# bcollico/Deep-Multiview-Depth-Estimation

Measured on AMD Instinct MI355X. Metric: depth maps/sec + warp-kernel HBM GB/s, 3-view 640x512 D=192, 1/2/4/8 GPU, higher is better.
Workload: dtype f32

## Files before the change

deep-multiview-depth-estimation_amd/csrc/capi.hip:

```cpp
#include <algorithm>
#include <cmath>
#include <cstring>

#include "../../include/train/mvs_region_train.h"
#include "launchers.h"

namespace {

using mvs::Geometry;

int check_geometry(int B, int V, int C, int h, int w, int d_count, Geometry& g, int store_es = 0) {
  if (B <= 0 || C <= 0 || h < 2 || w < 2 || d_count <= 0) return MVS_ERR_INVALID_ARGUMENT;
  if (V < 1 || V > MVS_MAX_VIEWS) return MVS_ERR_UNSUPPORTED_VIEWS;
  const uint64_t hw = (uint64_t)h * (uint64_t)w;
  if ((uint64_t)C * hw >= (1ull << 31) || h > 32000 || w > 32000) return MVS_ERR_TOO_LARGE;
  const bool packed = V >= 2 && V <= 8;
  const uint64_t padded = (uint64_t)V * (uint64_t)((C + 3) / 4) * (uint64_t)(h + 2) * (uint64_t)(w + 2) * 16u;
  if (packed && (padded >= (1ull << 31) || 8ull * hw * (uint64_t)store_es >= (1ull << 32))) return MVS_ERR_TOO_LARGE;
  const uint64_t tiles = (hw + mvs::kBlock - 1) / mvs::kBlock;
  const uint64_t total = (uint64_t)B * tiles * (uint64_t)d_count;
  if (total >= (1ull << 31) - 8) return MVS_ERR_TOO_LARGE;
  g.B = B;
  g.V = V;
  g.C = C;
// ... 681 lines not shown
    return MVS_ERR_INVALID_ARGUMENT;
  if (rd <= 0 || rh <= 0 || rw <= 0 || d <= 0 || h <= 0 || w <= 0) return MVS_ERR_INVALID_ARGUMENT;
  if (x0d < 0 || x0h < 0 || x0w < 0 || pd < 0 || ph < 0 || pw < 0) return MVS_ERR_INVALID_ARGUMENT;
  if (!bn_all_or_none(bn_scale, bn_shift, bn_mean)) return MVS_ERR_INVALID_ARGUMENT;
  if ((uint64_t)batch * c_in * rd * rh * rw * 4u >= (1ull << 31)) return MVS_ERR_TOO_LARGE;
  const int layout = (flags & MVS_LAYOUT_CHANNELS_LAST) ? ((flags & MVS_DECONV_WEIGHT_TAPS) ? 3 : 1)
                                                        : ((flags & MVS_DECONV_WEIGHT_TAPS) ? 2 : 0);
  const mvs::LaunchCheck lc;
  mvs::launch_deconv3d_k3s2(x, x2, layout, batch, c_in, rd, rh, rw, x0d, x0h,
                            x0w, weight, d, h, w, pd, ph, pw, bn_scale, bn_shift, bn_mean, residual, y,
                            (hipStream_t)stream);
  return lc.status();
}

int mvs_conv3d_region_fwd(int mode, int flags, const float* x, const float* x2, const float* weight, float* y,
                          int batch, int c_in, int c_out, const int* dims, const int* out_origin,
                          const int* out_size, const int* in_origin, const int* in_size,
                          const int* pad, const float* bn_scale, const float* bn_shift,
                          const float* bn_mean, const unsigned* x_absmax, unsigned* y_bound, void* stream) {
  if (!x || !weight || !y || !dims || !out_origin || !out_size || batch <= 0) return MVS_ERR_INVALID_ARGUMENT;
  if ((uintptr_t)y_bound & 3u) return MVS_ERR_INVALID_ARGUMENT;
  if (mode < MVS_CONV_S1 || mode > MVS_CONV_T2 ||
      (flags & ~(MVS_CONV_OUT_NCDHW | MVS_CONV_IN_C4 | MVS_CONV_IN_BF16 | MVS_CONV_IN_SPLIT | MVS_CONV_PER_LANE |
                 MVS_CONV_S2_LDS)))
    return MVS_ERR_INVALID_ARGUMENT;
  if ((flags & MVS_CONV_S2_LDS) && (flags & MVS_CONV_PER_LANE)) return MVS_ERR_INVALID_ARGUMENT;
  if ((flags & MVS_CONV_IN_BF16) && !(flags & MVS_CONV_IN_C4)) return MVS_ERR_INVALID_ARGUMENT;
  if ((flags & MVS_CONV_IN_SPLIT) && (!(flags & MVS_CONV_IN_C4) || (flags & MVS_CONV_IN_BF16) || !x_absmax ||
                                      ((uintptr_t)x_absmax & 3u)))
    return MVS_ERR_INVALID_ARGUMENT;
  if ((flags & MVS_CONV_IN_C4) && (mode != MVS_CONV_S2 || c_in % 4)) return MVS_ERR_INVALID_ARGUMENT;
  if (mode != MVS_CONV_S2 && (!in_origin || !in_size)) return MVS_ERR_INVALID_ARGUMENT;
  if (!both_or_neither(in_origin, in_size)) return MVS_ERR_INVALID_ARGUMENT;
  const bool boxed = in_origin != nullptr;
  if (mode != MVS_CONV_S1 && !pad) return MVS_ERR_INVALID_ARGUMENT;
  if (((uintptr_t)x | (uintptr_t)x2 | (uintptr_t)weight) & 15u) return MVS_ERR_INVALID_ARGUMENT;
  if (!bn_all_or_none(bn_scale, bn_shift, bn_mean)) return MVS_ERR_INVALID_ARGUMENT;
  uint64_t ovox = (uint64_t)batch, ivox = (uint64_t)batch, nvox = (uint64_t)batch * c_in;
  for (int k = 0; k < 3; ++k) {
    if (dims[k] <= 0 || out_size[k] <= 0 || out_origin[k] < 0 || out_origin[k] + out_size[k] > dims[k])
      return MVS_ERR_INVALID_ARGUMENT;
    if (boxed && (in_size[k] <= 0 || in_origin[k] < 0 || in_origin[k] + in_size[k] > dims[k]))
      return MVS_ERR_INVALID_ARGUMENT;
    ovox *= (uint64_t)out_size[k];
    ivox *= (uint64_t)(boxed ? in_size[k] : dims[k]);
    nvox *= (uint64_t)dims[k];
  }
  uint64_t svox = 1;
  for (int k = 0; k < 3; ++k) svox *= (uint64_t)(boxed ? in_size[k] : dims[k]);
  const uint64_t desc_bytes = mode == MVS_CONV_S2 ? svox * 64u : svox * (uint64_t)c_in * 4u;
  if (ovox >= (1ull << 31) || desc_bytes >= 0xFFFFFFC0ull || ivox * (uint64_t)c_in >= (1ull << 62) ||
      nvox >= (1ull << 62))
    return MVS_ERR_TOO_LARGE;
  const mvs::LaunchCheck lc;
  const int quads = (flags & MVS_CONV_IN_C4)
                        ? ((flags & MVS_CONV_IN_SPLIT) ? 3 : ((flags & MVS_CONV_IN_BF16) ? 2 : 1)) : 0;
  const int st = mvs::launch_conv3d_region(mode, (flags & MVS_CONV_OUT_NCDHW) != 0, quads,
                                           x, x2, weight, y, batch, c_in, c_out, dims, out_origin, out_size,
                                           in_origin, in_size, pad, bn_scale, bn_shift, bn_mean,
                                           (hipStream_t)stream, reinterpret_cast<const uint32_t*>(x_absmax),
                                           reinterpret_cast<uint32_t*>(y_bound), (flags & MVS_CONV_PER_LANE) != 0,
                                           nullptr, nullptr, (flags & MVS_CONV_S2_LDS) != 0);
  if (st != MVS_OK) return st;
  return lc.status();
}

int mvs_conv3d_region_split_weights(const float* weight, int c_in, int c_out, unsigned short* frag, int* weight_exp) {
  if (!weight || !frag || !weight_exp) return MVS_ERR_INVALID_ARGUMENT;
  if (c_out <= 0 || c_out % 16 || !(c_in == 16 || (c_in > 0 && c_in % 32 == 0))) return MVS_ERR_INVALID_ARGUMENT;
  int ew;
  if (!split_scale(weight, (size_t)27 * c_out * c_in, &ew)) return MVS_ERR_INVALID_ARGUMENT;
  const int kbs = mvs::conv3d_region_split_kblocks(c_in), nbs = c_out / 16;
  for (int kb = 0; kb < kbs; ++kb)
    for (int nb = 0; nb < nbs; ++nb)
      for (int lane = 0; lane < 64; ++lane)
        for (int j = 0; j < 8; ++j) {
          const int c = lane & 15, gq = lane >> 4, co = nb * 16 + c;
          int tap, ci;
          if (c_in == 16) {
            tap = 2 * kb + (gq >> 1);
            ci = 8 * (gq & 1) + j;
          } else {
            tap = kb / (c_in / 32);
            ci = (kb % (c_in / 32)) * 32 + 8 * gq + j;
          }
// ... 173 lines not shown
```

deep-multiview-depth-estimation_amd/csrc/conv3d_region.hip:

```cpp
#include <cstdlib>

#include "launchers.h"
#include "region_conv.h"

namespace mvs {
namespace {

struct Geo {
  int n[3];
  int o0[3];
  int on[3];
  int i0[3];
  int in[3];
  int pad[3];
  int out_cf;
  int in_c4;
  const uint32_t* absmax;
  uint32_t* y_bound;
  int st0[3];
  int stn[3];
};

__device__ inline void store_out(float* __restrict__ y, const Geo& g, int b, int co, int vz, int vy, int vx,
                                 int CO, float v) {
  const size_t vox = ((size_t)(vz + g.st0[0]) * g.stn[1] + (vy + g.st0[1])) * g.stn[2] + (vx + g.st0[2]);
  const size_t rvol = (size_t)g.stn[0] * g.stn[1] * g.stn[2];
  if (g.out_cf) y[((size_t)b * CO + co) * rvol + vox] = v;
  else y[((size_t)b * rvol + vox) * CO + co] = v;
}

template <int MODE, int CI, int CO, int RB, int QM, int CLS, int PS = 1>
__device__ __forceinline__ void region_conv(
    const float* __restrict__ x, const float* __restrict__ x2, const float* __restrict__ w,
    float* __restrict__ y, const float* __restrict__ bn_scale, const float* __restrict__ bn_shift,
    const float* __restrict__ bn_mean, const Geo& g) {
  constexpr int NB = CO / 16;
  static_assert(CI % 16 == 0 && CO % 16 == 0, "channel counts in multiples of 16");
  static_assert((MODE == kT2) == (CLS >= 0), "parity classes: transposed convolutions");
  static_assert(PS == 1 || (PS == 4 && CI == 112), "partial sums: the 112-channel input gradient only");
  const int lane = (int)threadIdx.x & 63;
  const int m = lane & 15, kq = lane >> 4;
  const int b = (int)blockIdx.z;

  int cf[3], cn[3];
  constexpr int par[3] = {CLS >= 0 ? (CLS >> 2) & 1 : 0, CLS >= 0 ? (CLS >> 1) & 1 : 0, CLS >= 0 ? CLS & 1 : 0};
  if constexpr (MODE == kT2) {
#pragma unroll
    for (int d = 0; d < 3; ++d) class_dim(g.o0[d], g.on[d], g.pad[d], par[d], cf[d], cn[d]);
  } else {
#pragma unroll
    for (int d = 0; d < 3; ++d) {
      cf[d] = g.o0[d];
      cn[d] = g.on[d];
    }
// ... 27 lines not shown
      else bs[d] = ((o[d] + g.pad[d] - par[d]) >> 1) - g.i0[d];
      unsigned mk = 0;
#pragma unroll
      for (int tt = 0; tt < 3; ++tt) {
        const int dl = MODE == kT2 ? -(tt >> 1) : tt;
        const bool in = ok && bs[d] + dl >= 0 && bs[d] + dl < lim[d] && !(MODE == kT2 && ((tt & 1) != par[d]));
        mk |= in ? (1u << tt) : 0u;
      }
      vm[rb][d] = mk;
    }
    lin[rb] = (bs[0] * lim[1] + bs[1]) * lim[2] + bs[2];
  }

  f4v acc[PS][RB][NB];
#pragma unroll
  for (int ps = 0; ps < PS; ++ps)
#pragma unroll
    for (int rb = 0; rb < RB; ++rb)
#pragma unroll
      for (int nb = 0; nb < NB; ++nb) acc[ps][rb][nb] = f4v{0.0f, 0.0f, 0.0f, 0.0f};

  const size_t rvol = (size_t)g.in[0] * g.in[1] * g.in[2];
  const int sy = lim[2], sz = lim[1] * lim[2];
#pragma unroll
  for (int tz = 0; tz < 3; ++tz) {
    if (MODE == kT2 && ((tz & 1) != par[0])) continue;
#pragma unroll
    for (int ty = 0; ty < 3; ++ty) {
      if (MODE == kT2 && ((ty & 1) != par[1])) continue;
      const int dz = MODE == kT2 ? -(tz >> 1) : tz, dy = MODE == kT2 ? -(ty >> 1) : ty;
      uint32_t vox[3][RB];
#pragma unroll
      for (int tx = 0; tx < 3; ++tx)
#pragma unroll
        for (int rb = 0; rb < RB; ++rb) {
          const int dx = MODE == kT2 ? -(tx >> 1) : tx;
          const bool ok = ((vm[rb][0] >> tz) & (vm[rb][1] >> ty) & (vm[rb][2] >> tx) & 1u) != 0;
          vox[tx][rb] = ok ? (uint32_t)(lin[rb] + dz * sz + dy * sy + dx) : kOob;
        }
#pragma unroll
      for (int cb = 0; cb < CI / 16; ++cb) {
        const int c4 = cb * 16 + kq * 4;
        const int ps = PS == 1 ? 0 : (cb + 1) / 2;
        Rsrc rs, rs2;
        if constexpr (MODE == kS2) {
          if constexpr (QM == 2)
            rs = make_rsrc(reinterpret_cast<const char*>(x) + ((size_t)b * (CI / 4) + cb * 4) * rvol * 8,
                           (uint32_t)(rvol * 32));
          else if constexpr (QM == 1 || QM == 3)
            rs = make_rsrc(x + ((size_t)b * (CI / 4) + cb * 4) * rvol * 4, (uint32_t)(rvol * 64));
          else
            rs = make_rsrc(x + ((size_t)b * CI + cb * 16) * rvol, (uint32_t)(rvol * 64));
        } else {
          rs = make_rsrc(x + (size_t)b * rvol * CI, (uint32_t)(rvol * CI * 4));
          if (x2) rs2 = make_rsrc(x2 + (size_t)b * rvol * CI, (uint32_t)(rvol * CI * 4));
        }
        f4v a[3][RB], bw[3][NB];
#pragma unroll
        for (int tx = 0; tx < 3; ++tx) {
          if (MODE == kT2 && ((tx & 1) != par[2])) continue;
#pragma unroll
          for (int rb = 0; rb < RB; ++rb) {
            const uint32_t vx = vox[tx][rb];
            f4v v;
            if constexpr (MODE == kS2) {
              if constexpr (QM == 2) {
                typedef __attribute__((ext_vector_type(2))) unsigned v2u;
                const v2u p = __builtin_amdgcn_raw_buffer_load_b64(
                    rs, (int)(vx == kOob ? kOob : ((uint32_t)kq * (uint32_t)rvol + vx) * 8u), 0, 0);
                v = f4v{__uint_as_float(p.x << 16), __uint_as_float(p.x & 0xFFFF0000u),
                          __uint_as_float(p.y << 16), __uint_as_float(p.y & 0xFFFF0000u)};
              } else if constexpr (QM == 3) {
                v = unsplit4(__builtin_bit_cast(uint4, __builtin_amdgcn_raw_buffer_load_b128(
                                 rs, (int)(vx == kOob ? kOob : ((uint32_t)kq * (uint32_t)rvol + vx) * 16u), 0, 0)),
                             sx);
              } else if constexpr (QM == 1) {
                v = ld4(rs, vx == kOob ? kOob : ((uint32_t)kq * (uint32_t)rvol + vx) * 16u, 0);
              } else {
#pragma unroll
                for (int q = 0; q < 4; ++q)
                  v[q] = __uint_as_float(__builtin_amdgcn_raw_buffer_load_b32(
                      rs, (int)(vx == kOob ? kOob : ((uint32_t)(kq * 4 + q) * (uint32_t)rvol + vx) * 4u), 0, 0));
              }
            } else {
              const uint32_t eo = vx == kOob ? kOob : (vx * (uint32_t)CI + (uint32_t)c4) * 4u;
              v = ld4(rs, eo, 0);
              if (x2) v += ld4(rs2, eo, 0);
            }
            a[tx][rb] = v;
          }
          const float* wt = w + (size_t)((tz * 3 + ty) * 3 + tx) * CO * CI;
#pragma unroll
          for (int nb = 0; nb < NB; ++nb)
            bw[tx][nb] = *reinterpret_cast<const f4v*>(wt + (size_t)(nb * 16 + m) * CI + c4);
        }
#pragma unroll
        for (int tx = 0; tx < 3; ++tx) {
          if (MODE == kT2 && ((tx & 1) != par[2])) continue;
#pragma unroll
          for (int s = 0; s < 4; ++s)
#pragma unroll
            for (int rb = 0; rb < RB; ++rb)
#pragma unroll
              for (int nb = 0; nb < NB; ++nb)
                acc[ps][rb][nb] =
                    __builtin_amdgcn_mfma_f32_16x16x4f32(a[tx][rb][s], bw[tx][nb][s], acc[ps][rb][nb], 0, 0, 0);
        }
      }
    }
  }

  float vmax = 0.0f;
#pragma unroll
  for (int nb = 0; nb < NB; ++nb) {
    const int co = nb * 16 + m;
    const float sc = bn_scale ? bn_scale[co] : 1.0f, sh = bn_scale ? bn_shift[co] : 0.0f,
                mu = bn_scale ? bn_mean[co] : 0.0f;
#pragma unroll
    for (int rb = 0; rb < RB; ++rb)
#pragma unroll
      for (int r = 0; r < 4; ++r) {
        const int row = row0 + rb * 16 + kq * 4 + r;
        if (row >= rows) continue;
        const int jx = row % cn[2], t = row / cn[2];
        const int jy = t % cn[1], jz = t / cn[1];
        const int vz = cf[0] + step * jz - g.o0[0], vy = cf[1] + step * jy - g.o0[1],
                  vx = cf[2] + step * jx - g.o0[2];
        float v = acc[0][rb][nb][r];
        if constexpr (PS == 4)
          v = (v + acc[1][rb][nb][r]) + (acc[PS - 2][rb][nb][r] + acc[PS - 1][rb][nb][r]);
        if (bn_scale) v = fmaxf((v - mu) * sc + sh, 0.0f);
        vmax = fmaxf(vmax, fabsf(v));
        store_out(y, g, b, co, vz, vy, vx, CO, v);
      }
  }
  if (g.y_bound) bound_update(g.y_bound, vmax);
}

template <int MODE, int CI, int CO, int RB, int QM = 0, int PS = 1>
__global__ __launch_bounds__(kBlock) void conv3d_region_kernel(
    const float* __restrict__ x, const float* __restrict__ x2, const float* __restrict__ w,
    float* __restrict__ y, const float* __restrict__ bn_scale, const float* __restrict__ bn_shift,
    const float* __restrict__ bn_mean, Geo g) {
  if constexpr (MODE == kT2) {
    switch (blockIdx.y) {
#define MVS_T2_CLASS(c) \
  case c: region_conv<MODE, CI, CO, RB, QM, c, PS>(x, x2, w, y, bn_scale, bn_shift, bn_mean, g); break;
      MVS_T2_CLASS(0) MVS_T2_CLASS(1) MVS_T2_CLASS(2) MVS_T2_CLASS(3)
      MVS_T2_CLASS(4) MVS_T2_CLASS(5) MVS_T2_CLASS(6) MVS_T2_CLASS(7)
#undef MVS_T2_CLASS
      default: break;
    }
  } else {
    region_conv<MODE, CI, CO, RB, QM, -1, PS>(x, x2, w, y, bn_scale, bn_shift, bn_mean, g);
  }
}

template <int MODE, int CI, int CO, int RB, int QM = 0, int PS = 1>
void launch_mode(const float* x, const float* x2, const float* w, float* y, const float* sc, const float* sh,
                 const float* mu, int B, const Geo& g, hipStream_t s) {
  hipLaunchKernelGGL((conv3d_region_kernel<MODE, CI, CO, RB, QM, PS>), region_grid(MODE, RB, B, g.on), dim3(kBlock), 0, s,
                     x, x2, w, y, sc, sh, mu, g);
}

template <int CI>
struct S1TileF {
  static constexpr int TZ = CI == 16 ? 8 : (CI == 32 ? 4 : 2);
  static constexpr int PX = 18, PY = 6, PZ = TZ + 2, PV = PX * PY * PZ;
  static constexpr int NCH = CI / 4;
  static constexpr int REC = CI * 4;
  static constexpr int LDS = PV * REC;
};

template <int CI>
__device__ inline int s1f_off(int v, int c) {
  constexpr int NCH = CI / 4;
  return v * (CI * 4) + ((c ^ (((v * NCH) >> 3) % NCH)) << 4);
}

template <int CI, int CO>
__global__ __launch_bounds__(kBlock) void conv3d_s1_lds_kernel(
    const float* __restrict__ x, const float* __restrict__ w, float* __restrict__ y,
    const float* __restrict__ bn_scale, const float* __restrict__ bn_shift, const float* __restrict__ bn_mean, Geo g,
    int tiles_x, int tiles_y, int tiles_z) {
  using T = S1TileF<CI>;
// ... 105 lines not shown
      float v = acc[r][i];
      if (bn_scale) v = fmaxf((v - mu) * sc + sh, 0.0f);
      vmax = fmaxf(vmax, fabsf(v));
      store_out(y, g, b, co, tz0 + zz, ty0 + yy, tx0 + 4 * kq + i, CO, v);
    }
  }
  if (g.y_bound) bound_update(g.y_bound, vmax);
}

template <int CI>
void launch_s1_lds(const float* x, const float* w, float* y, const float* sc, const float* sh, const float* mu,
                   int B, const Geo& g, hipStream_t s) {
  const int tx = (g.on[2] + 15) / 16, ty = (g.on[1] + 3) / 4, tz = (g.on[0] + S1TileF<CI>::TZ - 1) / S1TileF<CI>::TZ;
  hipLaunchKernelGGL((conv3d_s1_lds_kernel<CI, CI>), tile_grid(tx * ty * tz, B), dim3(kBlock), 0, s, x, w, y, sc, sh,
                     mu, g, tx, ty, tz);
}

}

int launch_conv3d_region(int mode, bool out_cf, int in_c4, const float* x, const float* x2, const float* w,
                         float* y, int B, int CI, int CO, const int* n, const int* o0, const int* on, const int* i0,
                         const int* in, const int* pad, const float* bn_scale, const float* bn_shift,
                         const float* bn_mean, hipStream_t s, const uint32_t* absmax, uint32_t* y_bound,
                         bool per_lane, const int* st0, const int* stn, bool s2_lds) {
  Geo g;
  g.y_bound = y_bound;
  g.out_cf = out_cf ? 1 : 0;
  g.in_c4 = in_c4;
  g.absmax = absmax;
  for (int d = 0; d < 3; ++d) {
    g.n[d] = n[d];
    g.o0[d] = o0[d];
    g.on[d] = on[d];
    g.i0[d] = i0 ? i0[d] : 0;
    g.in[d] = in ? in[d] : n[d];
    g.pad[d] = pad ? pad[d] : 1;
    g.st0[d] = st0 ? st0[d] : 0;
    g.stn[d] = stn ? stn[d] : on[d];
  }
  static const bool s1_lds = [] {
    const char* e = getenv("MVS_FP32_S1_LDS");
    return e && e[0] == '1';
  }();
  if (mode == kS1 && !x2 && CI == CO && !per_lane && s1_lds) {
    if (CI == 16) return launch_s1_lds<16>(x, w, y, bn_scale, bn_shift, bn_mean, B, g, s), MVS_OK;
    if (CI == 32) return launch_s1_lds<32>(x, w, y, bn_scale, bn_shift, bn_mean, B, g, s), MVS_OK;
    if (CI == 64) return launch_s1_lds<64>(x, w, y, bn_scale, bn_shift, bn_mean, B, g, s), MVS_OK;
  }
  if (mode == kS2 && CI == 32 && CO == 16 && (in_c4 == 0 || in_c4 == 1) && !x2 && !absmax && !y_bound &&
      !per_lane && !st0 && !stn && !i0 && !in && !out_cf && pad && (s2_lds || conv_s2_lds_enabled()) &&
      (uint64_t)n[0] * (uint64_t)n[1] * (uint64_t)n[2] * 128u < 0xFFFFFFF0ull) {
    launch_conv_s2_lds(x, in_c4, w, y, B, n, o0, on, pad, bn_scale, bn_shift, bn_mean, s);
    return MVS_OK;
  }
  static const int s2_rb = [] {
    const char* e = getenv("MVS_S2_RB");
    return e && e[0] == '4' ? 4 : 2;
  }();
  if (mode == kS2 && in_c4 == 1 && CI == 32 && s2_rb == 4) {
    if (CO == 16) return launch_mode<kS2, 32, 16, 4, 1>(x, x2, w, y, bn_scale, bn_shift, bn_mean, B, g, s), MVS_OK;
    if (CO == 32) return launch_mode<kS2, 32, 32, 4, 1>(x, x2, w, y, bn_scale, bn_shift, bn_mean, B, g, s), MVS_OK;
  }
#define MVS_REGION_CASE(MD, A, C)                                                       \
  if (mode == MD && CI == A && CO == C) {                                               \
    launch_mode<MD, A, C, 2>(x, x2, w, y, bn_scale, bn_shift, bn_mean, B, g, s);        \
    return MVS_OK;                                                                      \
  }
#define MVS_REGION_S2(A, C)                                                                                   \
  if (mode == kS2 && CI == A && CO == C) {                                                                    \
    if (in_c4 == 3) launch_mode<kS2, A, C, 2, 3>(x, x2, w, y, bn_scale, bn_shift, bn_mean, B, g, s);         \
    else if (in_c4 == 2) launch_mode<kS2, A, C, 2, 2>(x, x2, w, y, bn_scale, bn_shift, bn_mean, B, g, s);    \
    else if (in_c4) launch_mode<kS2, A, C, 2, 1>(x, x2, w, y, bn_scale, bn_shift, bn_mean, B, g, s);         \
    else launch_mode<kS2, A, C, 2, 0>(x, x2, w, y, bn_scale, bn_shift, bn_mean, B, g, s);                    \
    return MVS_OK;                                                                                            \
  }
  MVS_REGION_S2(32, 16) MVS_REGION_S2(32, 32) MVS_REGION_S2(32, 64)
  MVS_REGION_CASE(kS1, 16, 16) MVS_REGION_CASE(kS1, 32, 32) MVS_REGION_CASE(kS1, 64, 64)
  static const int t2_rb = [] {
    const char* e = getenv("MVS_T2_RB");
    return e && e[0] == '4' ? 4 : e && e[0] == '2' ? 2 : 0;
  }();
  if (mode == kT2 && CI == 64 && CO == 32 && t2_rb == 4)
    return launch_mode<kT2, 64, 32, 4>(x, x2, w, y, bn_scale, bn_shift, bn_mean, B, g, s), MVS_OK;
  if (mode == kT2 && CI == 32 && CO == 16 && t2_rb != 2)
    return launch_mode<kT2, 32, 16, 4>(x, x2, w, y, bn_scale, bn_shift, bn_mean, B, g, s), MVS_OK;
  MVS_REGION_CASE(kT2, 64, 32) MVS_REGION_CASE(kT2, 32, 16)
#undef MVS_REGION_CASE
#undef MVS_REGION_S2
  return MVS_ERR_INVALID_ARGUMENT;
}

void launch_conv3d_s2_dgrad(const float* gy, const float* w27, float* gx, int B, const int* n, const int* pad_lo,
                            const int* out, hipStream_t s) {
  Geo g;
  g.y_bound = nullptr;
  g.absmax = nullptr;
  g.out_cf = 1;
  g.in_c4 = 0;
  for (int d = 0; d < 3; ++d) {
    g.n[d] = n[d];
    g.o0[d] = 0;
    g.on[d] = n[d];
    g.i0[d] = 0;
    g.in[d] = out[d];
    g.pad[d] = pad_lo[d];
    g.st0[d] = 0;
    g.stn[d] = n[d];
  }
// ... 5 lines not shown
```

deep-multiview-depth-estimation_amd/csrc/launchers.h:

```cpp
#pragma once

#include <hip/hip_runtime.h>

#include "common.h"

namespace mvs {

void launch_plane_sampling(const float* K, const float* R, const float* T, const float* d_min,
                           const float* d_int, int B, int V, int h, int w, int d_begin,
                           int d_count, float d_scale, float* sampling, hipStream_t s);

size_t packed_bytes(int B, int V, int C, int h, int w);
void launch_cost_volume_fwd(const Geometry& g, const float* feat, const Cams& cm, float* sampling,
                            float* packed, float* cv, hipStream_t s, hipEvent_t ev0 = nullptr,
                            hipEvent_t ev1 = nullptr);
void launch_cost_volume_fwd_c4(const Geometry& g, const float* feat, const Cams& cm, float* sampling,
                               float* packed, float* cv, hipStream_t s, hipEvent_t ev0 = nullptr,
                               hipEvent_t ev1 = nullptr, uint32_t* absmax = nullptr, bool split = false);
void launch_cost_volume_fwd_c4_bf16(const Geometry& g, const float* feat, const Cams& cm, float* sampling,
                                    float* packed, void* cv, hipStream_t s, hipEvent_t ev0 = nullptr,
                                    hipEvent_t ev1 = nullptr);
void launch_cost_volume_fwd_bf16(const Geometry& g, const float* feat, const Cams& cm, float* sampling,
                                 float* packed, void* cv, hipStream_t s, hipEvent_t ev0 = nullptr,
                                 hipEvent_t ev1 = nullptr);
// ... 60 lines not shown
                         const int* n, const int* o0, const int* on, const int* pad, const float* bn_scale,
                         const float* bn_shift, const float* bn_mean, hipStream_t s);

int launch_conv2d_narrow(const float* in, const float* wt, float* out, int N, int Cin, int Cout, int H, int W,
                         int K, int stride, const float* bn_scale, const float* bn_shift, const float* bn_mean,
                         uint32_t* y_bound, hipStream_t s);

int conv2d_split_kblocks(int c_in, int k);
int launch_conv2d_split(const float* x, const void* wfrag, int w_exp, float* y, int N, int Cin, int Cout, int H,
                        int W, int K, int stride, const float* bn_scale, const float* bn_shift, const float* bn_mean,
                        const uint32_t* x_bound, uint32_t* y_bound, hipStream_t s);

void launch_deconv3d_k3s2(const float* x, const float* x2, int layout, int B, int Cin, int rd,
                          int rh, int rw, int x0d, int x0h, int x0w, const float* weight, int D, int H,
                          int W, int pd, int ph, int pw, const float* bn_scale, const float* bn_shift,
                          const float* bn_mean, const float* residual, float* y, hipStream_t s);

int launch_conv3d_region(int mode, bool out_cf, int in_c4, const float* x, const float* x2, const float* w,
                         float* y, int B, int CI, int CO, const int* n, const int* o0, const int* on, const int* i0,
                         const int* in,
                         const int* pad, const float* bn_scale, const float* bn_shift, const float* bn_mean,
                         hipStream_t s, const uint32_t* absmax = nullptr, uint32_t* y_bound = nullptr,
                         bool per_lane = false, const int* st0 = nullptr, const int* stn = nullptr,
                         bool s2_lds = false);
void launch_conv_head_fp32(const float* cv4, int B, int D, int H, int W, const float* w0wz, const float* bn0_sc,
                           const float* bn0_sh, const float* bn0_mu, const float* w1, const float* w1p,
                           const float* bn1_sc, const float* bn1_sh, const float* bn1_mu, const int* pad,
                           const int* o0, const int* on, float* y0, float* y1, hipStream_t s,
                           hipEvent_t ev0 = nullptr, hipEvent_t ev1 = nullptr);
void launch_bn_train_params(const double* sums, int C, double count, const double* bu, const double* bcnt, int Cp,
                            int ncls, const float* prev, const float* w, const float* bias, float* rmean, float* rvar,
                            long long* nbt, double momentum, double eps, float* params, hipStream_t s);

int conv3d_region_split_kblocks(int c_in);
int launch_conv3d_region_split(int mode, bool out_cf, const float* x, const float* x2, const void* wfrag, int w_exp,
                               float* y, int B, int CI, int CO, const int* n, const int* o0, const int* on,
                               const int* i0, const int* in, const int* pad, const float* bn_scale,
                               const float* bn_shift, const float* bn_mean, const uint32_t* x_bound,
                               const uint32_t* x2_bound, uint32_t* y_bound, hipStream_t s, bool per_lane = false,
                               const float* y_addend = nullptr, const int* store_origin = nullptr,
                               const int* store_size = nullptr, double* stats = nullptr, float* y_mid = nullptr,
                               float* y_high = nullptr, const float* in_bn = nullptr);
long conv3d_region_split_slots(int mode, int B, int CI, int CO, const int* on, bool per_lane, bool has_x2,
                               bool in_bn = false);

size_t channel_stats_slots(bool channels_last, int B, int C, size_t voxels);
void launch_channel_stats(const float* x, bool channels_last, int B, int C, size_t voxels, double* stats,
// ... 12 lines not shown
```

deep-multiview-depth-estimation_amd/mvs_amd/_lib.py:

```python
import ctypes
import os

import torch

_HERE = os.path.dirname(os.path.abspath(__file__))
LIB_NAME = "libmvs_cost_volume.so"
LIB_PATH = os.environ.get("MVS_LIB_PATH") or os.path.join(_HERE, LIB_NAME)
ABI_VERSION = 24

MVS_OK = 0
MVS_BWD_DETERMINISTIC = 1
MVS_LAYOUT_CHANNELS_LAST = 1
MVS_CONV_S1, MVS_CONV_S2, MVS_CONV_T2 = 0, 1, 2
MVS_CONV_OUT_NCDHW = 1
MVS_CONV_PER_LANE = 32
MVS_CONV_S2_LDS = 256
MVS_CONV_SUM_INPUT = 64
MVS_CONV_IN_BN = 128
MVS_CONV_IN_C4 = 2
MVS_CONV_WINO_Z = 4
MVS_CONV_IN_BF16 = 8
MVS_CONV_IN_SPLIT = 16
MVS_DECONV_WEIGHT_TAPS = 2
STATUS = {0: "ok", -1: "invalid argument", -2: "unsupported n_views", -3: "too large",
          -4: "HIP runtime error"}

_c_int, _c_float, _p = ctypes.c_int, ctypes.c_float, ctypes.c_void_p

_CV_ARGS = [_p] * 6 + [_c_int] * 7 + [_c_float, _p, _p, _p]

SIGNATURES = {
    "mvs_abi_version": (_c_int, []),
    "mvs_status_string": (ctypes.c_char_p, [_c_int]),
    "mvs_sampling_workspace_bytes": (ctypes.c_size_t, [_c_int, _c_int]),
    "mvs_cost_volume_workspace_bytes": (ctypes.c_size_t, [_c_int, _c_int, _c_int, _c_int, _c_int,
                                                           _c_int]),
    "mvs_plane_sampling": (_c_int, [_p, _p, _p, _p, _p, _c_int, _c_int, _c_int, _c_int, _c_int,
                                    _c_int, _c_float, _p, _p]),
    "mvs_cost_volume_fwd": (_c_int, _CV_ARGS),
# ... 106 lines not shown
```

deep-multiview-depth-estimation_amd/mvs_amd/ops.py:

```python
import collections
import ctypes
import weakref
from typing import Optional

import torch

from . import _lib

_F32 = torch.float32


def _require_gpu(t, name):
    if not t.is_cuda:
        raise _lib.MVSLibraryError(
            "%s must be a GPU (HIP) tensor: the MI355X cost-volume path has no CPU fallback" % name)


def _eager_only(op, **side_outputs):
    given = [k for k, v in side_outputs.items() if v is not None]
    if given:
        raise NotImplementedError("mvs::%s writes %s in place (an undeclared mutation): eager mode only, not "
                                  "torch.compile / functionalization" % (op, ", ".join(given)))


# ... 947 lines not shown
    if _pipeline_lane() and torch.cuda.is_available():
        torch.cuda.current_stream().synchronize()
    return out


def _pipeline_lane():
    from . import streams
    return streams._LANE[0]


def clear_derived():
    _DERIVED.clear()


def region_weight(module):
    if isinstance(module, torch.nn.ConvTranspose3d):
        return derived("region_t", (module.weight,),
                       lambda w: w.permute(2, 3, 4, 1, 0).reshape(27, w.shape[1], w.shape[0]).contiguous())
    return derived("region", (module.weight,),
                   lambda w: w.permute(2, 3, 4, 0, 1).reshape(27, w.shape[0], w.shape[1]).contiguous())


@torch.library.custom_op("mvs::conv3d_region", mutates_args=())
def conv3d_region(x: torch.Tensor, x2: Optional[torch.Tensor], weight: torch.Tensor, mode: int,
                  dims: list[int], out_origin: list[int], out_size: list[int],
                  in_origin: Optional[list[int]], in_size: Optional[list[int]], pad: Optional[list[int]],
                  bn_scale: Optional[torch.Tensor] = None, bn_shift: Optional[torch.Tensor] = None,
                  bn_mean: Optional[torch.Tensor] = None, out_ncdhw: bool = False,
                  in_c4: bool = False, absmax: Optional[torch.Tensor] = None,
                  y_bound: Optional[torch.Tensor] = None, per_lane: bool = False,
                  s2_lds: bool = False) -> torch.Tensor:
    _require_gpu(x, "x")
    lib = _lib.load()
    quad_bf16 = in_c4 and x.dtype == torch.bfloat16
    quad_split = in_c4 and x.dtype == torch.int32
    if quad_split and (absmax is None or absmax.numel() != 8 or absmax.dtype != torch.int32):
        raise ValueError("the split cost volume needs its bound words (absmax, int32[8])")
    x = x.contiguous() if (quad_bf16 or quad_split) else x.to(_F32).contiguous()
    if x2 is not None:
        x2 = x2.to(_F32).contiguous()
    w = weight.to(device=x.device, dtype=_F32).contiguous()
    _, cout, cin = w.shape
    b = x.shape[0]
    bn, bp = _bn_triple(bn_scale, bn_shift, bn_mean, x.device)
    shape = (b, cout) + tuple(out_size) if out_ncdhw else (b,) + tuple(out_size) + (cout,)
    y = torch.empty(shape, device=x.device, dtype=_F32)
    flags = ((_lib.MVS_CONV_OUT_NCDHW if out_ncdhw else 0) | (_lib.MVS_CONV_IN_C4 if in_c4 else 0)
             | (_lib.MVS_CONV_IN_BF16 if quad_bf16 else 0) | (_lib.MVS_CONV_IN_SPLIT if quad_split else 0)
             | (_lib.MVS_CONV_PER_LANE if per_lane else 0) | (_lib.MVS_CONV_S2_LDS if s2_lds else 0))
    st = lib.mvs_conv3d_region_fwd(int(mode), flags, _lib.ptr(x), _opt_ptr(x2), _lib.ptr(w),
                                   _lib.ptr(y), b, cin, cout, _ints3(dims), _ints3(out_origin), _ints3(out_size),
                                   _opt_ints3(in_origin), _opt_ints3(in_size), _opt_ints3(pad), *bp,
                                   _lib.ptr(absmax.contiguous()) if quad_split else None,
                                   _bound_ptr(y_bound), _lib.stream_handle(x.device))
    _lib.check(st, "mvs_conv3d_region_fwd")
    return y


@conv3d_region.register_fake
def _(x, x2, weight, mode, dims, out_origin, out_size, in_origin, in_size, pad, bn_scale=None, bn_shift=None,
      bn_mean=None, out_ncdhw=False, in_c4=False, absmax=None, y_bound=None, per_lane=False, s2_lds=False):
    _eager_only("conv3d_region", y_bound=y_bound)
    if out_ncdhw:
        return x.new_empty((x.shape[0], weight.shape[1]) + tuple(out_size), dtype=_F32)
    return x.new_empty((x.shape[0],) + tuple(out_size) + (weight.shape[1],), dtype=_F32)


BOUND_WORDS = 2048


def bound_words(n, device):
    return torch.zeros((n, BOUND_WORDS), device=device, dtype=torch.int32)


def _bound_ptr(t):
    if t is None:
        return None
    if t.dtype != torch.int32 or t.numel() != BOUND_WORDS or not t.is_contiguous():
        raise ValueError("bound words: a contiguous int32 tensor of %d words" % BOUND_WORDS)
    return _lib.ptr(t)


# ... 272 lines not shown
```

include/mvs_cost_volume.h:

```cpp
#ifndef MVS_COST_VOLUME_H
#define MVS_COST_VOLUME_H

#include <stddef.h>

#ifdef __cplusplus
extern "C" {
#endif

#define MVS_ABI_VERSION 24

#define MVS_OK 0
#define MVS_ERR_INVALID_ARGUMENT (-1)
#define MVS_ERR_UNSUPPORTED_VIEWS (-2)
#define MVS_ERR_TOO_LARGE (-3)
#define MVS_ERR_HIP (-4)

#define MVS_MAX_VIEWS 16

int mvs_abi_version(void);

const char* mvs_status_string(int status);

size_t mvs_sampling_workspace_bytes(int n_images, int d_count);

// ... 140 lines not shown
                          int h, int w, int pd, int ph, int pw, const float* bn_scale,
                          const float* bn_shift, const float* bn_mean, const float* residual, float* y,
                          void* stream);

int mvs_conv_head_fp32_fwd(const float* cv4, int batch, int d, int h, int w, const float* w0_wz,
                           const float* bn0_scale, const float* bn0_shift, const float* bn0_mean, const float* w1,
                           const float* w1_pass, const float* bn1_scale, const float* bn1_shift,
                           const float* bn1_mean, const int* pad, const int* y1_origin, const int* y1_size,
                           float* y0, float* y1, void* stream, void* ev0, void* ev1);

#define MVS_CONV_S1 0
#define MVS_CONV_S2 1
#define MVS_CONV_T2 2
#define MVS_CONV_OUT_NCDHW 1

int mvs_conv3d_region_fwd(int mode, int flags, const float* x, const float* x2, const float* weight, float* y,
                          int batch, int c_in, int c_out, const int* dims, const int* out_origin,
                          const int* out_size, const int* in_origin, const int* in_size,
                          const int* pad, const float* bn_scale, const float* bn_shift,
                          const float* bn_mean, const unsigned* x_absmax, unsigned* y_bound, void* stream);

#define MVS_CONV_PER_LANE 32
#define MVS_CONV_S2_LDS 256

#define MVS_BOUND_WORDS 2048

int mvs_conv3d_region_split_weights(const float* weight, int c_in, int c_out, unsigned short* frag, int* weight_exp);

int mvs_conv3d_region_split_fwd(int mode, int flags, const float* x, const float* x2, const void* weight_frag,
                                int weight_exp, float* y, int batch, int c_in, int c_out, const int* dims,
                                const int* out_origin, const int* out_size, const int* in_origin, const int* in_size,
                                const int* pad, const float* bn_scale, const float* bn_shift, const float* bn_mean,
                                const unsigned* x_bound, const unsigned* x2_bound, unsigned* y_bound,
                                const float* y_addend, const int* store_origin, const int* store_size, double* stats,
                                float* y_mid, float* y_high, const float* in_bn, void* stream);

#define MVS_CONV_SUM_INPUT 64
#define MVS_CONV_IN_BN 128
long long mvs_conv3d_region_split_stats_slots(int mode, int flags, int batch, int c_in, int c_out,
                                              const int* out_size);

int mvs_softmax_depth_fwd(const float* x, int batch, int d_count, int h, int w, float* y, void* stream);

int mvs_depth_hypotheses_fwd(const float* d_min, const float* d_int, int batch, int d_num, float d_scale, float* out,
                             void* stream);

// ... 25 lines not shown
```

Measured before the change: 690.7.

## Share neighbouring x-tap activations across lanes via DPP row shifts in region conv

In the region 3D conv, when a 16-lane block's output voxels lie on one image row, the kernel now loads only the centre (or one) x-tap per lane and derives the neighbouring x-taps with DPP row shifts. Only the row-end lane loads its extra neighbour. This cuts the number of buffer loads per tap by up to two thirds. The shared path is the default, chosen per wave at runtime, and the old per-lane loads remain behind a new OWN_TAPS flag. The cost is extra template instantiations, a runtime branch, and added register pressure from the vend offsets.

```diff
diff --git a/deep-multiview-depth-estimation_amd/csrc/capi.hip b/deep-multiview-depth-estimation_amd/csrc/capi.hip
--- a/deep-multiview-depth-estimation_amd/csrc/capi.hip
+++ b/deep-multiview-depth-estimation_amd/csrc/capi.hip
@@ -727,7 +727,7 @@
   if ((uintptr_t)y_bound & 3u) return MVS_ERR_INVALID_ARGUMENT;
   if (mode < MVS_CONV_S1 || mode > MVS_CONV_T2 ||
       (flags & ~(MVS_CONV_OUT_NCDHW | MVS_CONV_IN_C4 | MVS_CONV_IN_BF16 | MVS_CONV_IN_SPLIT | MVS_CONV_PER_LANE |
-                 MVS_CONV_S2_LDS)))
+                 MVS_CONV_S2_LDS | MVS_CONV_OWN_TAPS)))
     return MVS_ERR_INVALID_ARGUMENT;
   if ((flags & MVS_CONV_S2_LDS) && (flags & MVS_CONV_PER_LANE)) return MVS_ERR_INVALID_ARGUMENT;
   if ((flags & MVS_CONV_IN_BF16) && !(flags & MVS_CONV_IN_C4)) return MVS_ERR_INVALID_ARGUMENT;
@@ -765,7 +765,8 @@
                                            in_origin, in_size, pad, bn_scale, bn_shift, bn_mean,
                                            (hipStream_t)stream, reinterpret_cast<const uint32_t*>(x_absmax),
                                            reinterpret_cast<uint32_t*>(y_bound), (flags & MVS_CONV_PER_LANE) != 0,
-                                           nullptr, nullptr, (flags & MVS_CONV_S2_LDS) != 0);
+                                           nullptr, nullptr, (flags & MVS_CONV_S2_LDS) != 0,
+                                           (flags & MVS_CONV_OWN_TAPS) != 0);
   if (st != MVS_OK) return st;
   return lc.status();
 }
diff --git a/deep-multiview-depth-estimation_amd/csrc/conv3d_region.hip b/deep-multiview-depth-estimation_amd/csrc/conv3d_region.hip
--- a/deep-multiview-depth-estimation_amd/csrc/conv3d_region.hip
+++ b/deep-multiview-depth-estimation_amd/csrc/conv3d_region.hip
@@ -1,4 +1,5 @@
 #include <cstdlib>
+#include <type_traits>
 
 #include "launchers.h"
 #include "region_conv.h"
@@ -29,7 +30,27 @@
   else y[((size_t)b * rvol + vox) * CO + co] = v;
 }
 
-template <int MODE, int CI, int CO, int RB, int QM, int CLS, int PS = 1>
+constexpr bool shared_taps(int mode, int ci, int qm, int ps) {
+  return ps == 1 && (mode == kS1 ? ci != 16 : mode == kT2 || qm == 1);
+}
+
+__device__ __forceinline__ bool block_on_one_line(int r0, int width, int rows) {
+  return r0 + 15 < rows && r0 % width + 15 < width;
+}
+
+constexpr int kRowShr1 = 0x111, kRowShl1 = 0x101;
+
+template <int CTRL>
+__device__ __forceinline__ f4v row_shift(const f4v& end, const f4v& src) {
+  f4v r;
+#pragma unroll
+  for (int q = 0; q < 4; ++q)
+    r[q] = __int_as_float(
+        __builtin_amdgcn_update_dpp(__float_as_int(end[q]), __float_as_int(src[q]), CTRL, 0xf, 0xf, false));
+  return r;
+}
+
+template <int MODE, int CI, int CO, int RB, int QM, int CLS, int PS = 1, bool OWN = true>
 __device__ __forceinline__ void region_conv(
     const float* __restrict__ x, const float* __restrict__ x2, const float* __restrict__ w,
     float* __restrict__ y, const float* __restrict__ bn_scale, const float* __restrict__ bn_shift,
@@ -103,6 +124,8 @@
 
   const size_t rvol = (size_t)g.in[0] * g.in[1] * g.in[2];
   const int sy = lim[2], sz = lim[1] * lim[2];
+  auto k_loop = [&](auto shared) __attribute__((always_inline)) {
+  constexpr bool SH = decltype(shared)::value;
 #pragma unroll
   for (int tz = 0; tz < 3; ++tz) {
     if (MODE == kT2 && ((tz & 1) != par[0])) continue;
@@ -119,6 +142,13 @@
           const bool ok = ((vm[rb][0] >> tz) & (vm[rb][1] >> ty) & (vm[rb][2] >> tx) & 1u) != 0;
           vox[tx][rb] = ok ? (uint32_t)(lin[rb] + dz * sz + dy * sy + dx) : kOob;
         }
+      uint32_t vend[RB];
+#pragma unroll
+      for (int rb = 0; rb < RB; ++rb) {
+        if constexpr (MODE == kS1) vend[rb] = m == 0 ? vox[0][rb] : m == 15 ? vox[2][rb] : kOob;
+        else if constexpr (MODE == kS2) vend[rb] = m == 15 ? vox[2][rb] : kOob;
+        else vend[rb] = m == 0 ? vox[2][rb] : kOob;
+      }
 #pragma unroll
       for (int cb = 0; cb < CI / 16; ++cb) {
         const int c4 = cb * 16 + kq * 4;
@@ -136,44 +166,60 @@
           rs = make_rsrc(x + (size_t)b * rvol * CI, (uint32_t)(rvol * CI * 4));
           if (x2) rs2 = make_rsrc(x2 + (size_t)b * rvol * CI, (uint32_t)(rvol * CI * 4));
         }
+        auto load_a = [&](uint32_t vx) __attribute__((always_inline)) {
+          f4v v;
+          if constexpr (MODE == kS2) {
+            if constexpr (QM == 2) {
+              typedef __attribute__((ext_vector_type(2))) unsigned v2u;
+              const v2u p = __builtin_amdgcn_raw_buffer_load_b64(
+                  rs, (int)(vx == kOob ? kOob : ((uint32_t)kq * (uint32_t)rvol + vx) * 8u), 0, 0);
+              v = f4v{__uint_as_float(p.x << 16), __uint_as_float(p.x & 0xFFFF0000u),
+                        __uint_as_float(p.y << 16), __uint_as_float(p.y & 0xFFFF0000u)};
+            } else if constexpr (QM == 3) {
+              v = unsplit4(__builtin_bit_cast(uint4, __builtin_amdgcn_raw_buffer_load_b128(
+                               rs, (int)(vx == kOob ? kOob : ((uint32_t)kq * (uint32_t)rvol + vx) * 16u), 0, 0)),
+                           sx);
+            } else if constexpr (QM == 1) {
+              v = ld4(rs, vx == kOob ? kOob : ((uint32_t)kq * (uint32_t)rvol + vx) * 16u, 0);
+            } else {
+#pragma unroll
+              for (int q = 0; q < 4; ++q)
+                v[q] = __uint_as_float(__builtin_amdgcn_raw_buffer_load_b32(
+                    rs, (int)(vx == kOob ? kOob : ((uint32_t)(kq * 4 + q) * (uint32_t)rvol + vx) * 4u), 0, 0));
+            }
+          } else {
+            const uint32_t eo = vx == kOob ? kOob : (vx * (uint32_t)CI + (uint32_t)c4) * 4u;
+            v = ld4(rs, eo, 0);
+            if (x2) v += ld4(rs2, eo, 0);
+          }
+          return v;
+        };
         f4v a[3][RB], bw[3][NB];
 #pragma unroll
         for (int tx = 0; tx < 3; ++tx) {
           if (MODE == kT2 && ((tx & 1) != par[2])) continue;
-#pragma unroll
-          for (int rb = 0; rb < RB; ++rb) {
-            const uint32_t vx = vox[tx][rb];
-            f4v v;
-            if constexpr (MODE == kS2) {
-              if constexpr (QM == 2) {
-                typedef __attribute__((ext_vector_type(2))) unsigned v2u;
-                const v2u p = __builtin_amdgcn_raw_buffer_load_b64(
-                    rs, (int)(vx == kOob ? kOob : ((uint32_t)kq * (uint32_t)rvol + vx) * 8u), 0, 0);
-                v = f4v{__uint_as_float(p.x << 16), __uint_as_float(p.x & 0xFFFF0000u),
-                          __uint_as_float(p.y << 16), __uint_as_float(p.y & 0xFFFF0000u)};
-              } else if constexpr (QM == 3) {
-                v = unsplit4(__builtin_bit_cast(uint4, __builtin_amdgcn_raw_buffer_load_b128(
-                                 rs, (int)(vx == kOob ? kOob : ((uint32_t)kq * (uint32_t)rvol + vx) * 16u), 0, 0)),
-                             sx);
-              } else if constexpr (QM == 1) {
-                v = ld4(rs, vx == kOob ? kOob : ((uint32_t)kq * (uint32_t)rvol + vx) * 16u, 0);
-              } else {
-#pragma unroll
-                for (int q = 0; q < 4; ++q)
-                  v[q] = __uint_as_float(__builtin_amdgcn_raw_buffer_load_b32(
-                      rs, (int)(vx == kOob ? kOob : ((uint32_t)(kq * 4 + q) * (uint32_t)rvol + vx) * 4u), 0, 0));
-              }
-            } else {
-              const uint32_t eo = vx == kOob ? kOob : (vx * (uint32_t)CI + (uint32_t)c4) * 4u;
-              v = ld4(rs, eo, 0);
-              if (x2) v += ld4(rs2, eo, 0);
-            }
-            a[tx][rb] = v;
-          }
+          const bool formed = SH && (MODE == kS1 ? tx != 1 : tx == 2);
+#pragma unroll
+          for (int rb = 0; rb < RB; ++rb)
+            if (!formed) a[tx][rb] = load_a(vox[tx][rb]);
           const float* wt = w + (size_t)((tz * 3 + ty) * 3 + tx) * CO * CI;
 #pragma unroll
           for (int nb = 0; nb < NB; ++nb)
             bw[tx][nb] = *reinterpret_cast<const f4v*>(wt + (size_t)(nb * 16 + m) * CI + c4);
+        }
+        if constexpr (SH && (MODE != kT2 || par[2] == 0)) {
+#pragma unroll
+          for (int rb = 0; rb < RB; ++rb) {
+            const f4v e = load_a(vend[rb]);
+            if constexpr (MODE == kS1) {
+              a[0][rb] = row_shift<kRowShr1>(e, a[1][rb]);
+              a[2][rb] = row_shift<kRowShl1>(e, a[1][rb]);
+            } else if constexpr (MODE == kS2) {
+              a[2][rb] = row_shift<kRowShl1>(e, a[0][rb]);
+            } else {
+              a[2][rb] = row_shift<kRowShr1>(e, a[0][rb]);
+            }
+          }
         }
 #pragma unroll
         for (int tx = 0; tx < 3; ++tx) {
@@ -189,6 +235,16 @@
         }
       }
     }
+  }
+  };
+  if constexpr (!OWN && shared_taps(MODE, CI, QM, PS)) {
+    bool all = true;
+#pragma unroll
+    for (int rb = 0; rb < RB; ++rb) all = all && block_on_one_line(row0 + rb * 16, cn[2], rows);
+    if (__builtin_amdgcn_readfirstlane((int)all)) k_loop(std::true_type{});
+    else k_loop(std::false_type{});
+  } else {
+    k_loop(std::false_type{});
   }
 
   float vmax = 0.0f;
@@ -218,7 +274,7 @@
   if (g.y_bound) bound_update(g.y_bound, vmax);
 }
 
-template <int MODE, int CI, int CO, int RB, int QM = 0, int PS = 1>
+template <int MODE, int CI, int CO, int RB, int QM = 0, int PS = 1, bool OWN = true>
 __global__ __launch_bounds__(kBlock) void conv3d_region_kernel(
     const float* __restrict__ x, const float* __restrict__ x2, const float* __restrict__ w,
     float* __restrict__ y, const float* __restrict__ bn_scale, const float* __restrict__ bn_shift,
@@ -226,22 +282,30 @@
   if constexpr (MODE == kT2) {
     switch (blockIdx.y) {
 #define MVS_T2_CLASS(c) \
-  case c: region_conv<MODE, CI, CO, RB, QM, c, PS>(x, x2, w, y, bn_scale, bn_shift, bn_mean, g); break;
+  case c: region_conv<MODE, CI, CO, RB, QM, c, PS, OWN>(x, x2, w, y, bn_scale, bn_shift, bn_mean, g); break;
       MVS_T2_CLASS(0) MVS_T2_CLASS(1) MVS_T2_CLASS(2) MVS_T2_CLASS(3)
       MVS_T2_CLASS(4) MVS_T2_CLASS(5) MVS_T2_CLASS(6) MVS_T2_CLASS(7)
 #undef MVS_T2_CLASS
       default: break;
     }
   } else {
-    region_conv<MODE, CI, CO, RB, QM, -1, PS>(x, x2, w, y, bn_scale, bn_shift, bn_mean, g);
+    region_conv<MODE, CI, CO, RB, QM, -1, PS, OWN>(x, x2, w, y, bn_scale, bn_shift, bn_mean, g);
   }
 }
 
 template <int MODE, int CI, int CO, int RB, int QM = 0, int PS = 1>
 void launch_mode(const float* x, const float* x2, const float* w, float* y, const float* sc, const float* sh,
-                 const float* mu, int B, const Geo& g, hipStream_t s) {
-  hipLaunchKernelGGL((conv3d_region_kernel<MODE, CI, CO, RB, QM, PS>), region_grid(MODE, RB, B, g.on), dim3(kBlock), 0, s,
-                     x, x2, w, y, sc, sh, mu, g);
+                 const float* mu, int B, const Geo& g, hipStream_t s, bool own_taps = true) {
+  const dim3 grid = region_grid(MODE, RB, B, g.on);
+  if constexpr (shared_taps(MODE, CI, QM, PS)) {
+    if (!own_taps) {
+      hipLaunchKernelGGL((conv3d_region_kernel<MODE, CI, CO, RB, QM, PS, false>), grid, dim3(kBlock), 0, s, x, x2, w, y,
+                         sc, sh, mu, g);
+      return;
+    }
+  }
+  hipLaunchKernelGGL((conv3d_region_kernel<MODE, CI, CO, RB, QM, PS, true>), grid, dim3(kBlock), 0, s, x, x2, w, y, sc,
+                     sh, mu, g);
 }
 
 template <int CI>
@@ -393,7 +457,7 @@
                          float* y, int B, int CI, int CO, const int* n, const int* o0, const int* on, const int* i0,
                          const int* in, const int* pad, const float* bn_scale, const float* bn_shift,
                          const float* bn_mean, hipStream_t s, const uint32_t* absmax, uint32_t* y_bound,
-                         bool per_lane, const int* st0, const int* stn, bool s2_lds) {
+                         bool per_lane, const int* st0, const int* stn, bool s2_lds, bool own_taps) {
   Geo g;
   g.y_bound = y_bound;
   g.out_cf = out_cf ? 1 : 0;
@@ -429,20 +493,20 @@
     return e && e[0] == '4' ? 4 : 2;
   }();
   if (mode == kS2 && in_c4 == 1 && CI == 32 && s2_rb == 4) {
-    if (CO == 16) return launch_mode<kS2, 32, 16, 4, 1>(x, x2, w, y, bn_scale, bn_shift, bn_mean, B, g, s), MVS_OK;
-    if (CO == 32) return launch_mode<kS2, 32, 32, 4, 1>(x, x2, w, y, bn_scale, bn_shift, bn_mean, B, g, s), MVS_OK;
+    if (CO == 16) return launch_mode<kS2, 32, 16, 4, 1>(x, x2, w, y, bn_scale, bn_shift, bn_mean, B, g, s, own_taps), MVS_OK;
+    if (CO == 32) return launch_mode<kS2, 32, 32, 4, 1>(x, x2, w, y, bn_scale, bn_shift, bn_mean, B, g, s, own_taps), MVS_OK;
   }
 #define MVS_REGION_CASE(MD, A, C)                                                       \
   if (mode == MD && CI == A && CO == C) {                                               \
-    launch_mode<MD, A, C, 2>(x, x2, w, y, bn_scale, bn_shift, bn_mean, B, g, s);        \
+    launch_mode<MD, A, C, 2>(x, x2, w, y, bn_scale, bn_shift, bn_mean, B, g, s, own_taps);        \
     return MVS_OK;                                                                      \
   }
 #define MVS_REGION_S2(A, C)                                                                                   \
   if (mode == kS2 && CI == A && CO == C) {                                                                    \
-    if (in_c4 == 3) launch_mode<kS2, A, C, 2, 3>(x, x2, w, y, bn_scale, bn_shift, bn_mean, B, g, s);         \
-    else if (in_c4 == 2) launch_mode<kS2, A, C, 2, 2>(x, x2, w, y, bn_scale, bn_shift, bn_mean, B, g, s);    \
-    else if (in_c4) launch_mode<kS2, A, C, 2, 1>(x, x2, w, y, bn_scale, bn_shift, bn_mean, B, g, s);         \
-    else launch_mode<kS2, A, C, 2, 0>(x, x2, w, y, bn_scale, bn_shift, bn_mean, B, g, s);                    \
+    if (in_c4 == 3) launch_mode<kS2, A, C, 2, 3>(x, x2, w, y, bn_scale, bn_shift, bn_mean, B, g, s, own_taps);         \
+    else if (in_c4 == 2) launch_mode<kS2, A, C, 2, 2>(x, x2, w, y, bn_scale, bn_shift, bn_mean, B, g, s, own_taps);    \
+    else if (in_c4) launch_mode<kS2, A, C, 2, 1>(x, x2, w, y, bn_scale, bn_shift, bn_mean, B, g, s, own_taps);         \
+    else launch_mode<kS2, A, C, 2, 0>(x, x2, w, y, bn_scale, bn_shift, bn_mean, B, g, s, own_taps);                    \
     return MVS_OK;                                                                                            \
   }
   MVS_REGION_S2(32, 16) MVS_REGION_S2(32, 32) MVS_REGION_S2(32, 64)
@@ -452,9 +516,9 @@
     return e && e[0] == '4' ? 4 : e && e[0] == '2' ? 2 : 0;
   }();
   if (mode == kT2 && CI == 64 && CO == 32 && t2_rb == 4)
-    return launch_mode<kT2, 64, 32, 4>(x, x2, w, y, bn_scale, bn_shift, bn_mean, B, g, s), MVS_OK;
+    return launch_mode<kT2, 64, 32, 4>(x, x2, w, y, bn_scale, bn_shift, bn_mean, B, g, s, own_taps), MVS_OK;
   if (mode == kT2 && CI == 32 && CO == 16 && t2_rb != 2)
-    return launch_mode<kT2, 32, 16, 4>(x, x2, w, y, bn_scale, bn_shift, bn_mean, B, g, s), MVS_OK;
+    return launch_mode<kT2, 32, 16, 4>(x, x2, w, y, bn_scale, bn_shift, bn_mean, B, g, s, own_taps), MVS_OK;
   MVS_REGION_CASE(kT2, 64, 32) MVS_REGION_CASE(kT2, 32, 16)
 #undef MVS_REGION_CASE
 #undef MVS_REGION_S2
diff --git a/deep-multiview-depth-estimation_amd/csrc/launchers.h b/deep-multiview-depth-estimation_amd/csrc/launchers.h
--- a/deep-multiview-depth-estimation_amd/csrc/launchers.h
+++ b/deep-multiview-depth-estimation_amd/csrc/launchers.h
@@ -106,7 +106,7 @@
                          const int* pad, const float* bn_scale, const float* bn_shift, const float* bn_mean,
                          hipStream_t s, const uint32_t* absmax = nullptr, uint32_t* y_bound = nullptr,
                          bool per_lane = false, const int* st0 = nullptr, const int* stn = nullptr,
-                         bool s2_lds = false);
+                         bool s2_lds = false, bool own_taps = false);
 void launch_conv_head_fp32(const float* cv4, int B, int D, int H, int W, const float* w0wz, const float* bn0_sc,
                            const float* bn0_sh, const float* bn0_mu, const float* w1, const float* w1p,
                            const float* bn1_sc, const float* bn1_sh, const float* bn1_mu, const int* pad,
diff --git a/deep-multiview-depth-estimation_amd/mvs_amd/_lib.py b/deep-multiview-depth-estimation_amd/mvs_amd/_lib.py
--- a/deep-multiview-depth-estimation_amd/mvs_amd/_lib.py
+++ b/deep-multiview-depth-estimation_amd/mvs_amd/_lib.py
@@ -15,6 +15,7 @@
 MVS_CONV_OUT_NCDHW = 1
 MVS_CONV_PER_LANE = 32
 MVS_CONV_S2_LDS = 256
+MVS_CONV_OWN_TAPS = 512
 MVS_CONV_SUM_INPUT = 64
 MVS_CONV_IN_BN = 128
 MVS_CONV_IN_C4 = 2
diff --git a/deep-multiview-depth-estimation_amd/mvs_amd/ops.py b/deep-multiview-depth-estimation_amd/mvs_amd/ops.py
--- a/deep-multiview-depth-estimation_amd/mvs_amd/ops.py
+++ b/deep-multiview-depth-estimation_amd/mvs_amd/ops.py
@@ -993,14 +993,30 @@
 
 
 @torch.library.custom_op("mvs::conv3d_region", mutates_args=())
-def conv3d_region(x: torch.Tensor, x2: Optional[torch.Tensor], weight: torch.Tensor, mode: int,
-                  dims: list[int], out_origin: list[int], out_size: list[int],
-                  in_origin: Optional[list[int]], in_size: Optional[list[int]], pad: Optional[list[int]],
-                  bn_scale: Optional[torch.Tensor] = None, bn_shift: Optional[torch.Tensor] = None,
-                  bn_mean: Optional[torch.Tensor] = None, out_ncdhw: bool = False,
-                  in_c4: bool = False, absmax: Optional[torch.Tensor] = None,
-                  y_bound: Optional[torch.Tensor] = None, per_lane: bool = False,
-                  s2_lds: bool = False) -> torch.Tensor:
+def _conv3d_region_op(x: torch.Tensor, x2: Optional[torch.Tensor], weight: torch.Tensor, mode: int,
+                      dims: list[int], out_origin: list[int], out_size: list[int],
+                      in_origin: Optional[list[int]], in_size: Optional[list[int]], pad: Optional[list[int]],
+                      bn_scale: Optional[torch.Tensor] = None, bn_shift: Optional[torch.Tensor] = None,
+                      bn_mean: Optional[torch.Tensor] = None, out_ncdhw: bool = False,
+                      in_c4: bool = False, absmax: Optional[torch.Tensor] = None,
+                      y_bound: Optional[torch.Tensor] = None, per_lane: bool = False,
+                      s2_lds: bool = False) -> torch.Tensor:
+    return _conv3d_region(x, x2, weight, mode, dims, out_origin, out_size, in_origin, in_size, pad, bn_scale,
+                          bn_shift, bn_mean, out_ncdhw, in_c4, absmax, y_bound, per_lane, s2_lds, False)
+
+
+def conv3d_region(x, x2, weight, mode, dims, out_origin, out_size, in_origin, in_size, pad, bn_scale=None,
+                  bn_shift=None, bn_mean=None, out_ncdhw=False, in_c4=False, absmax=None, y_bound=None,
+                  per_lane=False, s2_lds=False, own_taps=False):
+    if own_taps:
+        return _conv3d_region(x, x2, weight, mode, dims, out_origin, out_size, in_origin, in_size, pad, bn_scale,
+                              bn_shift, bn_mean, out_ncdhw, in_c4, absmax, y_bound, per_lane, s2_lds, True)
+    return _conv3d_region_op(x, x2, weight, mode, dims, out_origin, out_size, in_origin, in_size, pad, bn_scale,
+                             bn_shift, bn_mean, out_ncdhw, in_c4, absmax, y_bound, per_lane, s2_lds)
+
+
+def _conv3d_region(x, x2, weight, mode, dims, out_origin, out_size, in_origin, in_size, pad, bn_scale, bn_shift,
+                   bn_mean, out_ncdhw, in_c4, absmax, y_bound, per_lane, s2_lds, own_taps):
     _require_gpu(x, "x")
     lib = _lib.load()
     quad_bf16 = in_c4 and x.dtype == torch.bfloat16
@@ -1018,7 +1034,8 @@
     y = torch.empty(shape, device=x.device, dtype=_F32)
     flags = ((_lib.MVS_CONV_OUT_NCDHW if out_ncdhw else 0) | (_lib.MVS_CONV_IN_C4 if in_c4 else 0)
              | (_lib.MVS_CONV_IN_BF16 if quad_bf16 else 0) | (_lib.MVS_CONV_IN_SPLIT if quad_split else 0)
-             | (_lib.MVS_CONV_PER_LANE if per_lane else 0) | (_lib.MVS_CONV_S2_LDS if s2_lds else 0))
+             | (_lib.MVS_CONV_PER_LANE if per_lane else 0) | (_lib.MVS_CONV_S2_LDS if s2_lds else 0)
+             | (_lib.MVS_CONV_OWN_TAPS if own_taps else 0))
     st = lib.mvs_conv3d_region_fwd(int(mode), flags, _lib.ptr(x), _opt_ptr(x2), _lib.ptr(w),
                                    _lib.ptr(y), b, cin, cout, _ints3(dims), _ints3(out_origin), _ints3(out_size),
                                    _opt_ints3(in_origin), _opt_ints3(in_size), _opt_ints3(pad), *bp,
@@ -1028,7 +1045,7 @@
     return y
 
 
-@conv3d_region.register_fake
+@_conv3d_region_op.register_fake
 def _(x, x2, weight, mode, dims, out_origin, out_size, in_origin, in_size, pad, bn_scale=None, bn_shift=None,
       bn_mean=None, out_ncdhw=False, in_c4=False, absmax=None, y_bound=None, per_lane=False, s2_lds=False):
     _eager_only("conv3d_region", y_bound=y_bound)
diff --git a/include/mvs_cost_volume.h b/include/mvs_cost_volume.h
--- a/include/mvs_cost_volume.h
+++ b/include/mvs_cost_volume.h
@@ -186,6 +186,7 @@
 
 #define MVS_CONV_PER_LANE 32
 #define MVS_CONV_S2_LDS 256
+#define MVS_CONV_OWN_TAPS 512
 
 #define MVS_BOUND_WORDS 2048
 
```

Result: no change. 696.0, median of 6 (+0.8%).
